# LouisNUST/pose-unsupervised

Hardware: AMD Instinct MI355X
Metric: 4-view 256x256 frames/sec (fwd+triangulate) (higher is better)
Workload: dtype bf16

## Files before the change

### include/posu.h

```cpp
#ifndef POSU_H_
#define POSU_H_

#ifdef __cplusplus
extern "C" {
#endif

#define POSU_OK 0
#define POSU_ERR_ARG 1
#define POSU_ERR_HIP 2

#define POSU_F32 0
#define POSU_BF16 1
#define POSU_F64 2
#define POSU_F16 3
#define POSU_F16X3 4

const char* posu_last_error(void);
int posu_abi_version(void);

int posu_pack_nchw_to_nhwc(int dtype, const float* x, int N, int C, int H, int W,
                           void* y, int Cpad, int hflip, void* stream);

int posu_pack_s2d_nchw(int dtype, const float* x, int N, int C, int H, int W,
                       void* y, int Cpad, int hflip, void* stream);
// ... 51 lines not shown
                                          const float* s2, const float* b2, const float* s3, const float* b3,
                                          void* y, const float* s1n, const float* b1n, void* t1n, void* stream);
int posu_bottleneck_down_tail_stream_fwd(int dtype, const void* t1, const void* x, int N, int H, int W, int C,
                                         int P, const void* wstream, long long wstream_bytes, const float* s2,
                                         const float* b2, const float* s3, const float* b3, void* y,
                                         const float* s1n, const float* b1n, void* t1n, void* stream);

int posu_bottleneck_s2_tail_fwd(int dtype, const void* t1, const void* x, int N, int H, int W, int C, int P,
                                const void* wstream, long long wstream_bytes, const float* s2, const float* b2,
                                const float* shift, int Cout, void* y, void* stream);

int posu_bottleneck_s2_tail_next_fwd(int dtype, const void* t1, const void* x, int N, int H, int W, int C, int P,
                                     const void* wstream, long long wstream_bytes, const float* s2, const float* b2,
                                     const float* shift, int Cout, void* y, const float* s1n, const float* b1n,
                                     void* t1n, void* stream);

int posu_bottleneck_down_fwd(int dtype, const void* x, int N, int H, int W, int C, int P,
                             const void* w1, const float* s1, const float* b1, const void* w2,
                             const float* s2, const float* b2, const void* w3d, const float* shift3,
                             void* y, void* stream);

int posu_pack_view_rows(int dtype, const float* src, int V, int M, int HW, void* dst, void* stream);
int posu_gemm_rows_f32(int dtype, const void* x, int M, int K, const void* wt, int Ncol, int vblk,
                       float* out, void* stream);

int posu_deconv4x4s2_head_fwd(int dtype, const void* x, int N, int H, int W, int C,
                              const void* w, int Cout, const float* scale, const float* shift,
                              void* y, const void* hw, const void* hw_lo, int J, const float* hbias,
                              float* hm, void* stream);

// ... 238 lines not shown
```

### pose-unsupervised_amd/csrc/tail_common.h

```cpp
#pragma once
#include <string>

#include "gemm_common.h"

namespace posu {
namespace {

struct TailGeom {
  const void* t1;
  const void* x;
  void* y;
  const uint4* wst;
  const float* s2;
  const float* b2;
  const float* s3;
  const float* b3;
  int N, H;
  const float* s1n;
  const float* b1n;
  void* t1n;
  long long wseg;
  int warm;
};

template <int D, int STEPS>
struct WStream {
  static constexpr int kD = D;
  const char* grp;
  int wlane;
  uint4 wa[D][2];
  __device__ __forceinline__ WStream(const uint4* wst, int cq, int lane)
      : grp(reinterpret_cast<const char*>(wst) + cq * (STEPS * 2 * 1024)), wlane(lane * 16) {}
  __device__ __forceinline__ const uint4* frag(int p, int j) const {
    return reinterpret_cast<const uint4*>(grp + (min(p, STEPS - 1) * 2 + j) * 1024 + wlane);
  }
  __device__ __forceinline__ void refill(int slot, int p) {
    wa[slot][0] = *frag(p, 0);
// ... 136 lines not shown
    } else {
#pragma unroll
      for (int i = 0; i < MT; ++i) {
#pragma unroll
        for (int j = 0; j < 2; ++j) O::mma(acc[i][j], ws.wa[s][j], b[d % NB][i]);
        if (NB == 1 && d + 1 < KT) b[0][i] = *at(i, d + 1);
      }
      ws.refill(s, p0 + d + kD);
    }
    __builtin_amdgcn_sched_barrier(0);
  }
}

inline int tail_operands(TailGeom& g, const std::string& what, const void* t1, const void* x, int N, int H,
                         const void* wstream, long long wstream_bytes, const float* s2, const float* b2,
                         const float* s3, const float* b3, void* y, const float* s1n, const float* b1n, void* t1n) {
  POSU_REQUIRE(t1 && x && wstream && s2 && b2 && b3 && y, what + ": null pointer");
  POSU_REQUIRE(x != y && t1 != y, what + ": the output must not alias an input");
  POSU_REQUIRE(!t1n || (s1n && b1n && t1n != y && t1n != x && t1n != t1),
               what + ": the next conv1 needs its BN and an output that aliases no other operand");
  g = TailGeom{t1, x, y, static_cast<const uint4*>(wstream), s2, b2, s3, b3, N, H, s1n, b1n, t1n, wstream_bytes / 64,
               warm_wgs(wstream_bytes)};
  return POSU_OK;
}

inline int tail_sizes(const TailGeom& g, const std::string& what, int hmult, long long act_bytes,
                      long long wstream_bytes, long long need) {
  POSU_REQUIRE(wstream_bytes == need, what + ": wstream holds " + std::to_string(wstream_bytes) + " bytes, the " +
                                          (g.t1n ? "chained" : "plain") + " tail reads " + std::to_string(need));
  POSU_REQUIRE(g.N > 0 && g.H > 0 && g.H % hmult == 0,
               what + ": H must be a positive multiple of " + std::to_string(hmult) + " (the tile rows)");
  POSU_REQUIRE(act_bytes < (1LL << 31) - 256, what + ": activation exceeds the 2 GiB addressing range");
  for (const void* p : {g.t1, g.x, static_cast<const void*>(g.y), static_cast<const void*>(g.wst),
                        static_cast<const void*>(g.s3), static_cast<const void*>(g.b3),
                        static_cast<const void*>(g.t1n), static_cast<const void*>(g.s1n),
                        static_cast<const void*>(g.b1n)})
    POSU_REQUIRE((reinterpret_cast<size_t>(p) & 15) == 0, what + ": pointers must be 16-byte aligned");
  return POSU_OK;
}

}
}
```

### pose-unsupervised_amd/csrc/tail_s2.hip

```cpp
#include "tail_common.h"

namespace posu {
namespace {

template <bool NEXT>
struct S2Cfg {
  static constexpr int kWin = 64, kC = 256, kP = 128, kCout = 512, kWout = 32;
  static constexpr int kRows = 4, kTW = 16, kNW = 4, kPx = kRows * kTW;
  static constexpr int kWR = 2 * kRows + 1, kWC = 2 * kTW + 1;
  static constexpr int kRowB = kP * 2;
  static constexpr int kXRowB = kC * 2;
  static constexpr int kWinInst = (kWR * kWC * kRowB + 1023) / 1024;
  static constexpr int kBN2 = kWinInst * 1024;
  static constexpr int kLds = kBN2 + 2 * kP * 4;
  static constexpr int kT2 = 0;
  static constexpr int kX = kT2 + kPx * kRowB;
  static constexpr int kShift = kX + kPx * kXRowB;
  static constexpr int kKT = kP / 32;
  static constexpr int kKX = kC / 32;
  static constexpr int kNC = kCout / (32 * kNW);
  static constexpr int kSteps2 = 9 * kKT, kStepsC = kKT + kKX + (NEXT ? kKT : 0);
  static constexpr int kSteps = kSteps2 + kNC * kStepsC;
  static constexpr int kYC = kShift + kCout * 4;
  static constexpr int kD = 4;
  static_assert(kYC + (NEXT ? kPx * kRowB : 0) <= kBN2, "t2, the x pixels, the shift (and the y chunk) fit over the window");
  static_assert(2 * kLds <= 160 * 1024, "two workgroups per CU");
  static_assert(kKT % kD == 0 && kKX % kD == 0 && kSteps2 % kD == 0 && kStepsC % kD == 0,
                "every block starts on ring slot 0");
};

template <typename T, bool NEXT>
__global__ __launch_bounds__(S2Cfg<NEXT>::kNW * 64, 2) void tail_s2_kernel(TailGeom g) {
  using O = Op<T>;
  using K = S2Cfg<NEXT>;
  constexpr int ES = 2, MT = K::kRows;
  __shared__ __attribute__((aligned(16))) char smem[K::kLds];
  const int tid = threadIdx.x;
  const int lane = tid & 63;
  const int r16 = lane & 15, q = lane >> 4;
  const int cq = __builtin_amdgcn_readfirstlane(tid >> 6);
  const unsigned lds0 = static_cast<unsigned>(reinterpret_cast<size_t>((__attribute__((address_space(3))) char*)smem));
  const int Hin = g.H, Hout = Hin / 2;
  const int tiles_x = K::kWout / K::kTW, tiles_y = Hout / K::kRows;
  const int n = blockIdx.x / (tiles_x * tiles_y);
  const int rem = blockIdx.x - n * tiles_x * tiles_y;
  const int R0 = (rem / tiles_x) * K::kRows, C0 = (rem % tiles_x) * K::kTW;
  float* bn2 = reinterpret_cast<float*>(smem + K::kBN2);
  for (int c = tid; c < K::kP; c += K::kNW * 64) {
    bn2[c] = g.s2[c];
    bn2[K::kP + c] = g.b2[c];
  }

  {
    const u32x4 t1s = make_srd(g.t1, g.N * Hin * K::kWin * K::kP * ES);
    const int sub = lane >> 4, pc = lane & 15;
#pragma unroll
    for (int k = 0; k < (K::kWinInst + K::kNW - 1) / K::kNW; ++k) {
      const int m = cq + K::kNW * k;
      if (m < K::kWinInst) {
        const int pix = 4 * m + sub;
        const int wr = pix / K::kWC, wc = pix - wr * K::kWC;
        const int yy = 2 * R0 - 1 + wr, xx = 2 * C0 - 1 + wc;
        const int lc = pc ^ (wc & 15);
        const bool ok = wr < K::kWR && static_cast<unsigned>(yy) < static_cast<unsigned>(Hin) &&
                        static_cast<unsigned>(xx) < static_cast<unsigned>(K::kWin);
        dma16(t1s, ok ? (((n * Hin + yy) * K::kWin + xx) * K::kP + 8 * lc) * ES : kOOB,
              lds0 + static_cast<unsigned>(m) * 1024u);
      }
    }
  }

  WStream<K::kD, K::kSteps> ws(g.wst, cq, lane);
  ws.start(g, K::kNW * 64);

  f32x4 acc[MT][2];
  f32x4 acc1[MT][2];
  const int c32 = 32 * cq + cpair(q);
  using Win = Stride2Addr<K::kRowB, K::kWC>;
  using T2 = RowsAddr<K::kRowB, K::kTW, K::kTW>;
  using XI = RowsAddr<K::kXRowB, K::kTW, K::kTW>;

  zero(acc);
#pragma unroll 1
  for (int t = 0; t < 9; ++t) {
    const int dy = t / 3, dx = t - 3 * (t / 3);
    kblock<O, K::kKT, 2>(acc, ws, K::kKT * t, Win(smem, dy, dx, r16, q));
  }
  lds_barrier();
  {
    const u32x4 xs = make_srd(g.x, g.N * Hin * K::kWin * K::kC * ES);
    const int sub = lane >> 5, pc = lane & 31;
#pragma unroll
    for (int k = 0; k < K::kPx / 2 / K::kNW; ++k) {
      const int m = cq + K::kNW * k;
      const int px = 2 * m + sub, i = px >> 4, r = px & 15;
      const int lc = (pc & 16) | ((pc ^ r) & 15);
      dma16(xs, (((n * Hin + 2 * (R0 + i)) * K::kWin + 2 * (C0 + r)) * K::kC + 8 * lc) * ES,
            lds0 + static_cast<unsigned>(K::kX + m * 1024));
    }
  }
  {
// ... 6 lines not shown
    for (int i = 0; i < MT; ++i) {
      float v[8];
      pair(acc, i, v);
      bn_relu(v, sc, sh, nullptr);
      lds_store8<O, K::kRowB>(smem + K::kT2, 16 * i + r16, r16, c32 >> 3, v);
    }
  }
  vm_wait<0>();
  lds_barrier();

  const float* shl = reinterpret_cast<const float*>(smem + K::kShift);
  T* yg = reinterpret_cast<T*>(g.y);
  if constexpr (NEXT) zero(acc1);
#pragma unroll
  for (int nc = 0; nc < K::kNC; ++nc) {
    const int p0 = K::kSteps2 + K::kStepsC * nc;
    zero(acc);
    kblock<O, K::kKT, 2>(acc, ws, p0, T2(smem + K::kT2, r16, r16, q));
    kblock<O, K::kKX, 2>(acc, ws, p0 + K::kKT, XI(smem + K::kX, r16, r16, q));
    const int c0 = 128 * nc + c32;
    float sh[8];
    ld8(shl + c0, sh);
    if constexpr (NEXT) {
      if (nc > 0) lds_barrier();
    }
#pragma unroll
    for (int i = 0; i < MT; ++i) {
      float v[8];
      pair(acc, i, v);
      add8<false>(v, sh);
#pragma unroll
// ... 17 lines not shown
      float v[8];
      pair(acc1, i, v);
      bn_relu(v, sc, sh, nullptr);
      const size_t pix = (static_cast<size_t>(n) * Hout + R0 + i) * K::kWout + C0 + r16;
      *reinterpret_cast<uint4*>(tg + pix * K::kP + c32) = O::store_vals(v);
    }
  }
}

}
}

using namespace posu;

namespace {
int s2_tail_impl(const char* name, int dtype, const void* t1, const void* x, int N, int H, int W, int C, int P,
                 const void* wstream, long long wstream_bytes, const float* s2, const float* b2, const float* shift,
                 int Cout, void* y, const float* s1n, const float* b1n, void* t1n, void* stream) {
  const std::string what = name;
  const bool next = t1n != nullptr;
  using K = S2Cfg<false>;
  POSU_REQUIRE(dtype == POSU_BF16 || dtype == POSU_F16, what + ": dtype must be BF16 or F16");
  TailGeom g;
  if (int e = tail_operands(g, what, t1, x, N, H, wstream, wstream_bytes, s2, b2, nullptr, shift, y, s1n, b1n, t1n))
    return e;
  POSU_REQUIRE(W == K::kWin && C == K::kC && P == K::kP && Cout == K::kCout,
               what + ": built for the first Bottleneck of layer2 of PoseResNet at 256x256 (input W = 64, C = 256, "
                      "planes = 128, output channels 512)");
  const long long need = static_cast<long long>(K::kNW) * (next ? S2Cfg<true>::kSteps : K::kSteps) * 2 * 1024;
  if (int e = tail_sizes(g, what, 2 * K::kRows, static_cast<long long>(N) * H * W * C * 2, wstream_bytes, need))
    return e;
  const dim3 grid(static_cast<unsigned>(N * (H / 2 / K::kRows) * (K::kWout / K::kTW)));
  hipStream_t s = as_stream(stream);
  if (dtype == POSU_BF16) {
    if (next) hipLaunchKernelGGL((tail_s2_kernel<uint16_t, true>), grid, dim3(K::kNW * 64), 0, s, g);
    else hipLaunchKernelGGL((tail_s2_kernel<uint16_t, false>), grid, dim3(K::kNW * 64), 0, s, g);
  } else {
    if (next) hipLaunchKernelGGL((tail_s2_kernel<f16_t, true>), grid, dim3(K::kNW * 64), 0, s, g);
    else hipLaunchKernelGGL((tail_s2_kernel<f16_t, false>), grid, dim3(K::kNW * 64), 0, s, g);
  }
  return check_launch(name);
}
}

extern "C" int posu_bottleneck_s2_tail_fwd(int dtype, const void* t1, const void* x, int N, int H, int W, int C,
                                           int P, const void* wstream, long long wstream_bytes, const float* s2,
                                           const float* b2, const float* shift, int Cout, void* y, void* stream) {
  return s2_tail_impl("posu_bottleneck_s2_tail_fwd", dtype, t1, x, N, H, W, C, P, wstream, wstream_bytes, s2, b2,
                      shift, Cout, y, nullptr, nullptr, nullptr, stream);
}

extern "C" int posu_bottleneck_s2_tail_next_fwd(int dtype, const void* t1, const void* x, int N, int H, int W, int C,
                                                int P, const void* wstream, long long wstream_bytes, const float* s2,
                                                const float* b2, const float* shift, int Cout, void* y,
                                                const float* s1n, const float* b1n, void* t1n, void* stream) {
  if (!t1n) {
    set_error("posu_bottleneck_s2_tail_next_fwd: null pointer (t1n)");
    return POSU_ERR_ARG;
  }
  return s2_tail_impl("posu_bottleneck_s2_tail_next_fwd", dtype, t1, x, N, H, W, C, P, wstream, wstream_bytes, s2,
                      b2, shift, Cout, y, s1n, b1n, t1n, stream);
}
```

### pose-unsupervised_amd/lib/posu/_native.py

```python
import ctypes
import os
import threading

import torch

F32 = 0
BF16 = 1
F64 = 2
F16 = 3
F16X3 = 4

ABI_VERSION = 16

_LIB_PATH = os.path.join(os.path.dirname(os.path.abspath(__file__)), 'libposeu.so')
_lock = threading.Lock()
_lib = None

_p = ctypes.c_void_p
_i = ctypes.c_int
_f = ctypes.c_float
_ll = ctypes.c_longlong
_d = ctypes.c_double

_SIGNATURES = {
# ... 6 lines not shown
    'posu_nhwc_to_nchw_f32': [_i, _p, _i, _i, _i, _i, _p, _p],
    'posu_conv1x1_dual_fwd': [_i, _p, _i, _i, _i, _i, _p, _i, _i, _i, _i, _p, _i, _p, _p, _i, _p, _i, _p],
    'posu_conv_bk': [_i],
    'posu_stem_pool_fwd': [_i, _p, _i, _i, _i, _i, _p, _p, _p, _p, _p],
    'posu_stem_pool_views_fwd': [_i, _p, _i, _i, _i, _i, _i, _p, _p, _p, _p, _p],
    'posu_bottleneck_fwd': [_i, _p, _i, _i, _i, _i, _i, _p, _p, _p, _p, _p, _p, _p, _p, _p, _p, _p],
    'posu_bottleneck_tail_stream_fwd': [_i, _p, _p, _i, _i, _i, _i, _i, _p, _ll, _p, _p, _p, _p, _p, _p],
    'posu_bottleneck_tail_stream_next_fwd': [_i, _p, _p, _i, _i, _i, _i, _i, _p, _ll, _p, _p, _p, _p, _p, _p, _p,
                                             _p, _p],
    'posu_bottleneck_tail_stream_chain_fwd': [_i, _p, _p, _i, _i, _i, _i, _i, _i, _p, _ll, _p, _p, _p, _p, _p, _p,
                                              _p, _p, _p],
    'posu_bottleneck_down_tail_stream_fwd': [_i, _p, _p, _i, _i, _i, _i, _i, _p, _ll, _p, _p, _p, _p, _p, _p, _p,
                                             _p, _p],
    'posu_bottleneck_s2_tail_fwd': [_i, _p, _p, _i, _i, _i, _i, _i, _p, _ll, _p, _p, _p, _i, _p, _p],
    'posu_bottleneck_s2_tail_next_fwd': [_i, _p, _p, _i, _i, _i, _i, _i, _p, _ll, _p, _p, _p, _i, _p, _p, _p, _p, _p],
    'posu_bottleneck_down_fwd': [_i, _p, _i, _i, _i, _i, _i, _p, _p, _p, _p, _p, _p, _p, _p, _p, _p],
    'posu_conv2d_fwd': [_i, _p, _i, _i, _i, _i, _p, _i, _i, _i, _i, _i, _p, _p, _p, _i, _p, _i, _i, _i, _p],
    'posu_deconv4x4s2_fwd': [_i, _p, _i, _i, _i, _i, _p, _i, _p, _p, _i, _p, _i, _p],
    'posu_deconv4x4s2_head_fwd': [_i, _p, _i, _i, _i, _i, _p, _i, _p, _p, _p, _p, _p, _i, _p, _p, _p],
    'posu_head1x1_nchw_fwd': [_i, _p, _i, _i, _i, _i, _p, _i, _p, _p, _p],
    'posu_maxpool3x3s2_fwd': [_i, _p, _i, _i, _i, _i, _p, _p],
    'posu_softargmax2d_fwd': [_p, _i, _i, _i, _i, _f, _p, _p, _p, _p],
    'posu_softargmax2d_bwd': [_p, _p, _i, _i, _i, _i, _f, _p, _p, _p, _p],
    'posu_argmax2d_fwd': [_p, _i, _i, _i, _i, _i, _p, _p, _p, _p],
    'posu_affine2d_apply': [_p, _p, _i, _i, _i, _p, _p],
    'posu_epipolar_loss_fwd': [_p, _p, _p, _p, _i, _i, _i, _i, _p, _p, _p],
    'posu_epipolar_loss_bwd': [_p, _p, _p, _p, _i, _i, _i, _i, _p, _p, _p],
    'posu_triangulate_dlt': [_p, _p, _p, _i, _i, _i, _p, _i, _i, _i, _i, _p, _p],
    'posu_joints_mse_fwd': [_p, _p, _p, _i, _i, _i, _p, _p, _p],
    'posu_joints_mse_bwd': [_p, _p, _p, _i, _i, _i, _p, _p, _p],
# ... 138 lines not shown
```

### pose-unsupervised_amd/lib/posu/ops.py

```python
import numpy as np
import torch

from . import _native as nat
from ._native import F32, BF16, F64, F16, F16X3, ptr, call, stream_of, require_cuda

_TORCH_OF = {F32: torch.float32, BF16: torch.bfloat16, F16: torch.float16, F16X3: torch.float16}


def dtype_code(dtype):
    if dtype in ('bf16', torch.bfloat16, BF16):
        return BF16
    if dtype in ('fp32', 'f32', torch.float32, F32):
        return F32
    if dtype in ('fp16', 'f16', torch.float16, F16):
        return F16
    if dtype in ('fp16x3', F16X3):
        return F16X3
    raise ValueError('unsupported compute dtype %r (bf16 | fp16 | fp16x3 | fp32)' % (dtype,))


def torch_dtype(code):
    return _TORCH_OF[code]


# ... 99 lines not shown
    call('posu_bottleneck_s2_tail_fwd', code, ptr(t1), ptr(x), n, h, w, c, t1.shape[3], ptr(wstream),
         wstream.numel() * wstream.element_size(), ptr(s2), ptr(b2), ptr(shift), shift.numel(), ptr(out),
         stream_of(x.device))
    return out


def bottleneck_s2_tail_next_nhwc(t1, x, wstream, s2, b2, shift, s1n, b1n, code, out=None, t1n=None):
    n, h, w, c = x.shape
    if out is None:
        out = torch.empty((n, h // 2, w // 2, shift.numel()), dtype=x.dtype, device=x.device)
    if t1n is None:
        t1n = torch.empty((n, h // 2, w // 2, s1n.numel()), dtype=x.dtype, device=x.device)
    call('posu_bottleneck_s2_tail_next_fwd', code, ptr(t1), ptr(x), n, h, w, c, t1.shape[3], ptr(wstream),
         wstream.numel() * wstream.element_size(), ptr(s2), ptr(b2), ptr(shift), shift.numel(), ptr(out), ptr(s1n),
         ptr(b1n), ptr(t1n), stream_of(x.device))
    return out, t1n


def bottleneck_tail_stream_next_nhwc(t1, x, wstream, s2, b2, s3, b3, s1n, b1n, code, out=None, t1n=None):
    n, h, w, c = x.shape
    p = t1.shape[3]
    if out is None:
        out = torch.empty_like(x)
    if t1n is None:
        t1n = torch.empty((n, h, w, p), dtype=x.dtype, device=x.device)
    cm = cmul(code)
    call('posu_bottleneck_tail_stream_next_fwd', code, ptr(t1), ptr(x), n, h, w, c // cm, p // cm, ptr(wstream),
         wstream.numel() * wstream.element_size(), ptr(s2), ptr(b2), ptr(s3), ptr(b3), ptr(out), ptr(s1n), ptr(b1n),
         ptr(t1n), stream_of(x.device))
    return out, t1n
# ... 855 lines not shown
```

### pose-unsupervised_amd/lib/posu/packing.py

```python
import numpy as np
import torch

COUT_ALIGN = 64


def round_up(x, m):
    return (x + m - 1) // m * m


def pack_conv_weight(w, cin_pad, bk, dtype):
    cout, cin, kh, kw = w.shape
    k = kh * kw * cin_pad
    wt = torch.zeros((cout, kh, kw, cin_pad), dtype=torch.float32, device=w.device)
    wt[..., :cin] = w.detach().float().permute(0, 2, 3, 1)
    out = torch.zeros((round_up(cout, COUT_ALIGN), round_up(k, bk)), dtype=torch.float32, device=w.device)
    out[:cout, :k] = wt.reshape(cout, k)
    return out.to(dtype).contiguous()


def mfma_fragments(wpk):
    co, k = wpk.shape
    return wpk.reshape(co // 16, 16, k // 32, 4, 8).permute(0, 2, 3, 1, 4).reshape(co // 16, k // 32, 64, 8)


def pack_s2_tail_stream(w2pk, wdual, w1n=None):
    if tuple(w2pk.shape) != (128, 1152) or tuple(wdual.shape) != (512, 384):
        raise ValueError('pack_s2_tail_stream: conv2 pack [128][1152] and dual pack [512][384] expected, got %s / %s'
                         % (tuple(w2pk.shape), tuple(wdual.shape)))
    f2 = mfma_fragments(w2pk)
    s2 = f2.reshape(4, 2, 36, 64, 8).permute(0, 2, 1, 3, 4)
    fd = mfma_fragments(wdual)
    sd = fd.reshape(4, 4, 2, 12, 64, 8).permute(1, 0, 3, 2, 4, 5)
    if w1n is None:
        return torch.cat([s2, sd.reshape(4, 48, 2, 64, 8)], dim=1).contiguous()
    if tuple(w1n.shape) != (128, 512):
        raise ValueError('pack_s2_tail_stream: the next conv1 pack must be [128][512], got %s' % (tuple(w1n.shape),))
    f1 = mfma_fragments(w1n)
    s1 = f1.reshape(4, 2, 4, 4, 64, 8).permute(0, 2, 3, 1, 4, 5)
    sdn = torch.cat([sd, s1], dim=2)
    return torch.cat([s2, sdn.reshape(4, 64, 2, 64, 8)], dim=1).contiguous()


def pack_tail_stream(w2pk, w3pk, w1n=None):
# ... 232 lines not shown
```

### pose-unsupervised_amd/lib/posu/plan.py

```python
from collections import namedtuple

import torch

from . import ops
from .packing import (fold_bn, pack_bottleneck_conv1_weight, pack_bottleneck_conv3_weight, pack_bottleneck_down_weight,
                      pack_conv_weight, pack_deconv4x4_weight, pack_down_tail_stream,
                      pack_dual_1x1_weight, pack_s2_tail_stream, pack_stem_fused_weight, pack_stem_s2d_weight,
                      pack_tail_stream, split_exponent, to_split)

STEM_CIN_PAD = 8
STEM_S2D_PAD = 16
SPLIT_PAD = 32


def _stem_pads(code):
    return (2 * SPLIT_PAD, SPLIT_PAD) if code == ops.F16X3 else (STEM_CIN_PAD, STEM_S2D_PAD)


def _pack(pk32, code):
    if code == ops.F16X3:
        e = split_exponent(pk32)
        return to_split(pk32, e), e
    return pk32.to(ops.torch_dtype(code)).contiguous(), 0

# ... 145 lines not shown
        self.scale = None if e == 0 else torch.full((self.cout,), 2.0 ** -e, device=self.shift.device)
        self.stride2 = dconv.stride[0]

    def __call__(self, mid, x, code, out=None):
        if out is None:
            out = torch.empty(tuple(mid.shape[:3]) + (self.cout * ops.cmul(code),), dtype=mid.dtype, device=mid.device)
        key = ('dual', code, tuple(mid.shape), tuple(x.shape), self.cout)
        return _tuned(key, self.cout, lambda t: ops.conv1x1_dual_nhwc(
            mid, x, self.stride2, self.w, self.cout, self.shift, True, code, out=out, tile=t, scale=self.scale))


FUSED_BOTTLENECK = True
S2_TAIL = True
CHAINED_TAILS = True
S2_CHAIN = True
TAIL_W24 = True
SPLIT_TAILS = True
TAIL_W96 = True
CHAIN_LAYERS = True
CHAIN_LAYERS_2B = False
CHUNKS_F16X3 = 2
EARLY_LAYERS = 2
_FUSED_MAX_BYTES = (1 << 31) - 256


def _fused_fits(x, cout):
    px = x.shape[0] * x.shape[1] * x.shape[2]
    es = x.element_size()
    return px * max(x.shape[3], cout) * es < _FUSED_MAX_BYTES

# ... 41 lines not shown
        ds = blk.downsample
        if ds is not None and len(names) == 3 and ds[0].kernel_size == (1, 1) and \
                blk.conv3.weight.shape[1] % bk == 0 and ds[0].weight.shape[1] % bk == 0:
            for nm in names[:2]:
                self.convs.append(_Conv(getattr(blk, nm), getattr(blk, 'bn' + nm[-1]), True, code, bk))
            self.dual = _DualTail(blk.conv3, blk.bn3, ds[0], ds[1], code)
            c2 = self.convs[1]
            if self._built_for('fused_down'):
                self.packs['fused_down'] = pack_bottleneck_down_weight(self.dual.w, 64)
            if self._built_for('down_tail'):
                self.packs['down_tail'] = pack_down_tail_stream(c2.w, self.dual.w)
                self.dscale = (self.dual.scale if self.dual.scale is not None else
                               torch.ones(self.dual.cout, device=self.dual.shift.device))
            if self._built_for('s2_tail'):
                self.packs['s2_tail'] = pack_s2_tail_stream(c2.w, self.dual.w)
            return
        for nm in names:
            self.convs.append(_Conv(getattr(blk, nm), getattr(blk, 'bn' + nm[-1]), True, code, bk))
        if ds is not None:
            self.down = _Conv(ds[0], ds[1], False, code, bk)
        if self._built_for('fused'):
            self.packs['fused'] = (pack_bottleneck_conv1_weight(blk.conv1.weight, ops.torch_dtype(code)),
                                   pack_bottleneck_conv3_weight(blk.conv3.weight, ops.torch_dtype(code)))
        self.kind = next((k for k in ('l1', 'l2', 'l3') if self._built_for(k)), None)
        if self.kind is not None:
            self.packs['tail'] = pack_tail_stream(self.convs[1].w, self.convs[2].w)

    def _built_for(self, kernel):
        g = _GEOMETRY[kernel]
        if self.down is not None or (self.dual is None) != (g.dual is None) or len(self.convs) != (2 if g.dual else 3):
# ... 10 lines not shown
    def _chains(self, how):
        return self.kind is not None and any(self.code in a.codes and how in a.chains
                                             for a in _GEOMETRY[self.kind].at)

    def link_next(self, nxt):
        c2 = self.convs[1]
        if self.kind is not None and self.kind == nxt.kind:
            self.chain = nxt.convs[0]
            self.packs['tail_next'] = pack_tail_stream(c2.w, self.convs[2].w, self.chain.w)
        elif 'down_tail' in self.packs and nxt.kind == 'l1':
            self.chain = nxt.convs[0]
            self.packs['down_tail_next'] = pack_down_tail_stream(c2.w, self.dual.w, self.chain.w)
        elif 's2_tail' in self.packs and nxt.kind == 'l2':
            self.chain = nxt.convs[0]
            self.packs['s2_tail_next'] = pack_s2_tail_stream(c2.w, self.dual.w, self.chain.w)

    def link_layer(self, first):
        if not (self._chains('layer') and (self.code in _SPLIT or CHAIN_LAYERS_2B) and first.dual is not None):
            return
        c1n = first.convs[0]
        planes = self.convs[1].cout
        if c1n.k == 1 and c1n.stride == 1 and c1n.cout == 2 * planes and tuple(c1n.w.shape)[1] == self.convs[0].w.shape[1]:
            self.xchain = c1n
            self.packs['tail_layer'] = pack_tail_stream(self.convs[1].w, self.convs[2].w, c1n.w)

    @property
    def cout(self):
        return self.dual.cout if self.dual is not None else self.convs[-1].cout

    def _at(self, kernel, x):
# ... 47 lines not shown
            c1, c2, c3 = cs
            w1f, w3f = self.packs['fused']
            return ops.bottleneck_nhwc(x, w1f, c1.scale, c1.shift, c2.w, c2.scale, c2.shift, w3f, c3.scale, c3.shift,
                                       code, out=out), None
        if variant == 'fused_down':
            c1, c2 = cs
            return ops.bottleneck_down_nhwc(x, c1.w, c1.scale, c1.shift, c2.w, c2.scale, c2.shift,
                                            self.packs['fused_down'], self.dual.shift, code, out=out), None
        if variant == 'down_tail':
            c1, c2 = cs
            s1n, b1n = (self.chain.scale, self.chain.shift) if chained else (None, None)
            return ops.bottleneck_down_tail_stream_nhwc(
                c1(x, code), x, self.packs['down_tail_next' if chained else 'down_tail'], c2.scale, c2.shift,
                self.dscale, self.dual.shift, code, s1n=s1n, b1n=b1n, out=out)
        if variant == 's2_tail':
            c1, c2 = cs
            if chained:
                n1 = self.chain
                return ops.bottleneck_s2_tail_next_nhwc(c1(x, code), x, self.packs['s2_tail_next'], c2.scale, c2.shift,
                                                        self.dual.shift, n1.scale, n1.shift, code, out=out)
            return ops.bottleneck_s2_tail_nhwc(c1(x, code), x, self.packs['s2_tail'], c2.scale, c2.shift,
                                               self.dual.shift, code, out=out), None
        if variant == 'dual':
            return self.dual(cs[1](cs[0](x, code) if t1 is None else t1, code), x, code, out=out), None
        res = self.down(x, code) if self.down is not None else x
        y = x
        for c in cs[:-1]:
            y = c(y, code)
        return cs[-1](y, code, residual=res, out=out), None

    def __call__(self, x, code, out=None):
        return self.run(x, code, out=out, chain=False)[0]


class _Deconv:
    __slots__ = ('w', 'scale', 'shift', 'cout')

    def __init__(self, dc, bn, code, bk):
        if dc.stride != (2, 2) or dc.padding != (1, 1) or dc.output_padding != (0, 0):
            raise NotImplementedError('deconv supported for kernel 4, stride 2, padding 1')
        self.w, e = _pack(pack_deconv4x4_weight(dc.weight, 32 if code == ops.F16X3 else bk, torch.float32), code)
        self.scale, self.shift = fold_bn(bn, dc.bias)
        self.scale = _unscale(self.scale, e)
        self.cout = dc.weight.shape[1]
# ... 235 lines not shown
```

### pose-unsupervised_amd/lib/posu/roofline.py

```python

_R50 = ((3, 64, 64, 256, 64), (4, 128, 256, 512, 64), (6, 256, 512, 1024, 32), (3, 512, 1024, 2048, 16))


def r50_256_launches(n=128, es=2, joints=17):
    out = []
    act = lambda hw, c: n * hw * hw * c * es
    wb = lambda *dims: es * _prod(dims)
    out.append(('stem_pool (4 views)', n * 3 * 256 * 256 * 4 + wb(64, 147), act(64, 64)))
    out.append(('layer1.0 bottleneck64 (down)', act(64, 64) + wb(64, 64) + wb(64, 576) + wb(256, 64) + wb(256, 64),
                act(64, 256)))
    for b in (1, 2):
        out.append(('layer1.%d bottleneck64' % b, act(64, 256) + wb(64, 256) + wb(64, 576) + wb(256, 64),
                    act(64, 256)))
    out.append(('layer2.0 conv1', act(64, 256) + wb(128, 256), act(64, 128)))
    out.append(('layer2.0 strided tail + layer2.1 conv1',
                act(64, 128) + act(32, 256) + wb(128, 1152) + wb(512, 384) + wb(128, 512),
                act(32, 512) + act(32, 128)))
    for b in (1, 2):
        out.append(('layer2.%d chained tail' % b, act(32, 128) + act(32, 512) + wb(128, 1152) + wb(512, 128) +
                    wb(128, 512), act(32, 512) + act(32, 128)))
    out.append(('layer2.3 tail', act(32, 128) + act(32, 512) + wb(128, 1152) + wb(512, 128), act(32, 512)))
    out.append(('layer3.0 conv1', act(32, 512) + wb(256, 512), act(32, 256)))
    out.append(('layer3.0 conv2 s2', act(32, 256) + wb(256, 2304), act(16, 256)))
    out.append(('layer3.0 conv3|down', act(16, 256) + act(16, 512) + wb(1024, 768), act(16, 1024)))
    out.append(('layer3.1 conv1', act(16, 1024) + wb(256, 1024), act(16, 256)))
    for b in (1, 2, 3, 4):
        out.append(('layer3.%d chained tail' % b, act(16, 256) + act(16, 1024) + wb(256, 2304) + wb(1024, 256) +
                    wb(256, 1024), act(16, 1024) + act(16, 256)))
    out.append(('layer3.5 tail', act(16, 256) + act(16, 1024) + wb(256, 2304) + wb(1024, 256), act(16, 1024)))
    out.append(('layer4.0 conv1', act(16, 1024) + wb(512, 1024), act(16, 512)))
    out.append(('layer4.0 conv2 s2', act(16, 512) + wb(512, 4608), act(8, 512)))
    out.append(('layer4.0 conv3|down', act(8, 512) + act(8, 1024) + wb(2048, 1536), act(8, 2048)))
# ... 90 lines not shown
```

Measured before the change: 56530.

## Fuse layer2.0 conv1 into the strided tail kernel with autotuned selection

Result: faster. 58010 (median of 6 runs) (+2.6%).

```diff
diff --git a/include/posu.h b/include/posu.h
--- a/include/posu.h
+++ b/include/posu.h
@@ -89,6 +89,16 @@
                                      const void* wstream, long long wstream_bytes, const float* s2, const float* b2,
                                      const float* shift, int Cout, void* y, const float* s1n, const float* b1n,
                                      void* t1n, void* stream);
+
+int posu_bottleneck_s2_front_tail_fwd(int dtype, const void* x, int N, int H, int W, int C, int P, const float* s1,
+                                      const float* b1, const void* wstream, long long wstream_bytes,
+                                      const float* s2, const float* b2, const float* shift, int Cout, void* y,
+                                      void* stream);
+int posu_bottleneck_s2_front_tail_next_fwd(int dtype, const void* x, int N, int H, int W, int C, int P,
+                                           const float* s1, const float* b1, const void* wstream,
+                                           long long wstream_bytes, const float* s2, const float* b2,
+                                           const float* shift, int Cout, void* y, const float* s1n,
+                                           const float* b1n, void* t1n, void* stream);
 
 int posu_bottleneck_down_fwd(int dtype, const void* x, int N, int H, int W, int C, int P,
                              const void* w1, const float* s1, const float* b1, const void* w2,
diff --git a/pose-unsupervised_amd/csrc/tail_common.h b/pose-unsupervised_amd/csrc/tail_common.h
--- a/pose-unsupervised_amd/csrc/tail_common.h
+++ b/pose-unsupervised_amd/csrc/tail_common.h
@@ -21,6 +21,8 @@
   void* t1n;
   long long wseg;
   int warm;
+  const float* s1;
+  const float* b1;
 };
 
 template <int D, int STEPS>
@@ -187,13 +189,14 @@
 
 inline int tail_operands(TailGeom& g, const std::string& what, const void* t1, const void* x, int N, int H,
                          const void* wstream, long long wstream_bytes, const float* s2, const float* b2,
-                         const float* s3, const float* b3, void* y, const float* s1n, const float* b1n, void* t1n) {
-  POSU_REQUIRE(t1 && x && wstream && s2 && b2 && b3 && y, what + ": null pointer");
+                         const float* s3, const float* b3, void* y, const float* s1n, const float* b1n, void* t1n,
+                         bool front = false, const float* s1 = nullptr, const float* b1 = nullptr) {
+  POSU_REQUIRE((front ? s1 && b1 : t1 != nullptr) && x && wstream && s2 && b2 && b3 && y, what + ": null pointer");
   POSU_REQUIRE(x != y && t1 != y, what + ": the output must not alias an input");
   POSU_REQUIRE(!t1n || (s1n && b1n && t1n != y && t1n != x && t1n != t1),
                what + ": the next conv1 needs its BN and an output that aliases no other operand");
   g = TailGeom{t1, x, y, static_cast<const uint4*>(wstream), s2, b2, s3, b3, N, H, s1n, b1n, t1n, wstream_bytes / 64,
-               warm_wgs(wstream_bytes)};
+               warm_wgs(wstream_bytes), s1, b1};
   return POSU_OK;
 }
 
@@ -207,7 +210,8 @@
   for (const void* p : {g.t1, g.x, static_cast<const void*>(g.y), static_cast<const void*>(g.wst),
                         static_cast<const void*>(g.s3), static_cast<const void*>(g.b3),
                         static_cast<const void*>(g.t1n), static_cast<const void*>(g.s1n),
-                        static_cast<const void*>(g.b1n)})
+                        static_cast<const void*>(g.b1n), static_cast<const void*>(g.s1),
+                        static_cast<const void*>(g.b1)})
     POSU_REQUIRE((reinterpret_cast<size_t>(p) & 15) == 0, what + ": pointers must be 16-byte aligned");
   return POSU_OK;
 }
diff --git a/pose-unsupervised_amd/csrc/tail_s2.hip b/pose-unsupervised_amd/csrc/tail_s2.hip
--- a/pose-unsupervised_amd/csrc/tail_s2.hip
+++ b/pose-unsupervised_amd/csrc/tail_s2.hip
@@ -3,7 +3,7 @@
 namespace posu {
 namespace {
 
-template <bool NEXT>
+template <bool NEXT, bool FRONT = false>
 struct S2Cfg {
   static constexpr int kWin = 64, kC = 256, kP = 128, kCout = 512, kWout = 32;
   static constexpr int kRows = 4, kTW = 16, kNW = 4, kPx = kRows * kTW;
@@ -20,19 +20,32 @@
   static constexpr int kKX = kC / 32;
   static constexpr int kNC = kCout / (32 * kNW);
   static constexpr int kSteps2 = 9 * kKT, kStepsC = kKT + kKX + (NEXT ? kKT : 0);
-  static constexpr int kSteps = kSteps2 + kNC * kStepsC;
+  static constexpr int kF = FRONT ? kKX : 0;
+  static constexpr int kWinPx = kWinInst * 1024 / kRowB, kGroups = (kWR * kWC + 16 * kRows - 1) / (16 * kRows);
+  static constexpr int kSteps = kF + kSteps2 + kNC * kStepsC;
   static constexpr int kYC = kShift + kCout * 4;
   static constexpr int kD = 4;
   static_assert(kYC + (NEXT ? kPx * kRowB : 0) <= kBN2, "t2, the x pixels, the shift (and the y chunk) fit over the window");
   static_assert(2 * kLds <= 160 * 1024, "two workgroups per CU");
-  static_assert(kKT % kD == 0 && kKX % kD == 0 && kSteps2 % kD == 0 && kStepsC % kD == 0,
+  static_assert(kKT % kD == 0 && kKX % kD == 0 && kSteps2 % kD == 0 && kStepsC % kD == 0 && kF % kD == 0,
                 "every block starts on ring slot 0");
 };
 
-template <typename T, bool NEXT>
+template <int KX>
+struct HeldW {
+  static constexpr int kD = KX;
+  uint4 wa[KX][2];
+  __device__ __forceinline__ void refill(int, int) {}
+};
+template <int RowB>
+__device__ __forceinline__ uint4* win_chunk(char* img, int pix, int wc, int c8) {
+  return reinterpret_cast<uint4*>(img + pix * RowB + ((c8 ^ (wc & 15)) << 4));
+}
+
+template <typename T, bool NEXT, bool FRONT = false>
 __global__ __launch_bounds__(S2Cfg<NEXT>::kNW * 64, 2) void tail_s2_kernel(TailGeom g) {
   using O = Op<T>;
-  using K = S2Cfg<NEXT>;
+  using K = S2Cfg<NEXT, FRONT>;
   constexpr int ES = 2, MT = K::kRows;
   __shared__ __attribute__((aligned(16))) char smem[K::kLds];
   const int tid = threadIdx.x;
@@ -51,7 +64,7 @@
     bn2[K::kP + c] = g.b2[c];
   }
 
-  {
+  if constexpr (!FRONT) {
     const u32x4 t1s = make_srd(g.t1, g.N * Hin * K::kWin * K::kP * ES);
     const int sub = lane >> 4, pc = lane & 15;
 #pragma unroll
@@ -71,20 +84,106 @@
   }
 
   WStream<K::kD, K::kSteps> ws(g.wst, cq, lane);
-  ws.start(g, K::kNW * 64);
+  if constexpr (!FRONT) ws.start(g, K::kNW * 64);
 
   f32x4 acc[MT][2];
   f32x4 acc1[MT][2];
   const int c32 = 32 * cq + cpair(q);
+
   using Win = Stride2Addr<K::kRowB, K::kWC>;
   using T2 = RowsAddr<K::kRowB, K::kTW, K::kTW>;
   using XI = RowsAddr<K::kXRowB, K::kTW, K::kTW>;
+
+  if constexpr (FRONT) {
+    constexpr int kGrpPx = 16 * MT, kGrpB = kGrpPx * K::kXRowB;
+    constexpr int kDma = kGrpB / 1024 / K::kNW;
+    static_assert(2 * kGrpB <= (K::kGroups - 1) * kGrpPx * K::kRowB, "both buffers below the last group's t1");
+    static_assert(K::kGroups * kGrpPx >= K::kWinPx, "the groups cover the window");
+    unsigned wv[kWarmLoads];
+    warm_issue(wv, g.wst, g.wseg, g.warm, K::kNW * 64);
+    HeldW<K::kKX> w1;
+#pragma unroll
+    for (int d = 0; d < K::kKX; ++d)
+#pragma unroll
+      for (int j = 0; j < 2; ++j) w1.wa[d][j] = *ws.frag(d, j);
+    float sc[8], sh[8];
+    ld8(g.s1 + c32, sc);
+    ld8(g.b1 + c32, sh);
+    const u32x4 xs = make_srd(g.x, g.N * Hin * K::kWin * K::kC * ES);
+    auto px_off = [&](int pix, int& wc) {
+      const int wr = pix / K::kWC;
+      wc = pix - wr * K::kWC;
+      const int yy = 2 * R0 - 1 + wr, xx = 2 * C0 - 1 + wc;
+      const bool ok = wr < K::kWR && static_cast<unsigned>(yy) < static_cast<unsigned>(Hin) &&
+                      static_cast<unsigned>(xx) < static_cast<unsigned>(K::kWin);
+      return ok ? ((n * Hin + yy) * K::kWin + xx) * K::kC * ES : kOOB;
+    };
+    auto stage = [&](int gr, int b) {
+      const int sub = lane >> 5, pc = lane & 31;
+#pragma unroll
+      for (int k = 0; k < kDma; ++k) {
+        const int m = cq + K::kNW * k;
+        const int px = 2 * m + sub, r = px & 15;
+        const int lc = (pc & 16) | ((pc ^ r) & 15);
+        int wc;
+        const int off = px_off(kGrpPx * gr + px, wc);
+        dma16(xs, off == kOOB ? kOOB : off + 8 * lc * ES, lds0 + static_cast<unsigned>(b * kGrpB + m * 1024));
+      }
+    };
+    warm_use(wv);
+#pragma unroll
+    for (int d = 0; d < K::kKX; ++d) asm volatile("" ::"v"(w1.wa[d][0].x), "v"(w1.wa[d][1].x));
+    asm volatile("" ::"v"(sc[0]), "v"(sc[4]), "v"(sh[0]), "v"(sh[4]));
+    stage(K::kGroups - 1, 0);
+    stage(K::kGroups - 2, 1);
+    uint4 held[K::kGroups][MT];
+#pragma unroll
+    for (int s = 0; s < K::kGroups; ++s) {
+      const int gr = K::kGroups - 1 - s;
+      if (s + 1 < K::kGroups) vm_wait<kDma>();
+      else vm_wait<0>();
+      lds_barrier();
+      zero(acc);
+      kblock<O, K::kKX, 2>(acc, w1, 0, XI(smem + (s & 1) * kGrpB, r16, r16, q));
+      lds_barrier();
+      if (s + 2 < K::kGroups) stage(gr - 2, s & 1);
+#pragma unroll
+      for (int i = 0; i < MT; ++i) {
+        float v[8];
+        pair(acc, i, v);
+        bn_relu(v, sc, sh, nullptr);
+        int wc;
+        const bool pad = px_off(kGrpPx * gr + 16 * i + r16, wc) == kOOB;
+#pragma unroll
+        for (int e = 0; e < 8; ++e) v[e] = pad ? 0.f : v[e];
+        held[s][i] = O::store_vals(v);
+      }
+      if (s == 0) {
+#pragma unroll
+        for (int i = 0; i < MT; ++i) {
+          const int pix = kGrpPx * gr + 16 * i + r16;
+          if (pix < K::kWinPx) *win_chunk<K::kRowB>(smem, pix, pix % K::kWC, c32 >> 3) = held[s][i];
+        }
+      }
+    }
+#pragma unroll
+    for (int d = 0; d < K::kD; ++d) ws.refill(d, K::kF + d);
+#pragma unroll
+    for (int s = 1; s < K::kGroups; ++s)
+#pragma unroll
+      for (int i = 0; i < MT; ++i) {
+        const int pix = kGrpPx * (K::kGroups - 1 - s) + 16 * i + r16;
+        *win_chunk<K::kRowB>(smem, pix, pix % K::kWC, c32 >> 3) = held[s][i];
+      }
+    vm_wait<0>();
+    lds_barrier();
+  }
 
   zero(acc);
 #pragma unroll 1
   for (int t = 0; t < 9; ++t) {
     const int dy = t / 3, dx = t - 3 * (t / 3);
-    kblock<O, K::kKT, 2>(acc, ws, K::kKT * t, Win(smem, dy, dx, r16, q));
+    kblock<O, K::kKT, 2>(acc, ws, K::kF + K::kKT * t, Win(smem, dy, dx, r16, q));
   }
   lds_barrier();
   {
@@ -121,7 +220,7 @@
   if constexpr (NEXT) zero(acc1);
 #pragma unroll
   for (int nc = 0; nc < K::kNC; ++nc) {
-    const int p0 = K::kSteps2 + K::kStepsC * nc;
+    const int p0 = K::kF + K::kSteps2 + K::kStepsC * nc;
     zero(acc);
     kblock<O, K::kKT, 2>(acc, ws, p0, T2(smem + K::kT2, r16, r16, q));
     kblock<O, K::kKX, 2>(acc, ws, p0 + K::kKT, XI(smem + K::kX, r16, r16, q));
@@ -169,31 +268,40 @@
 using namespace posu;
 
 namespace {
-int s2_tail_impl(const char* name, int dtype, const void* t1, const void* x, int N, int H, int W, int C, int P,
-                 const void* wstream, long long wstream_bytes, const float* s2, const float* b2, const float* shift,
-                 int Cout, void* y, const float* s1n, const float* b1n, void* t1n, void* stream) {
+template <typename T>
+void s2_launch(bool next, bool front, dim3 grid, dim3 block, hipStream_t s, const TailGeom& g) {
+  if (front) {
+    if (next) hipLaunchKernelGGL((tail_s2_kernel<T, true, true>), grid, block, 0, s, g);
+    else hipLaunchKernelGGL((tail_s2_kernel<T, false, true>), grid, block, 0, s, g);
+  } else {
+    if (next) hipLaunchKernelGGL((tail_s2_kernel<T, true>), grid, block, 0, s, g);
+    else hipLaunchKernelGGL((tail_s2_kernel<T, false>), grid, block, 0, s, g);
+  }
+}
+
+int s2_tail_impl(const char* name, int dtype, bool front, const void* t1, const float* s1, const float* b1,
+                 const void* x, int N, int H, int W, int C, int P, const void* wstream, long long wstream_bytes,
+                 const float* s2, const float* b2, const float* shift, int Cout, void* y, const float* s1n,
+                 const float* b1n, void* t1n, void* stream) {
   const std::string what = name;
   const bool next = t1n != nullptr;
   using K = S2Cfg<false>;
   POSU_REQUIRE(dtype == POSU_BF16 || dtype == POSU_F16, what + ": dtype must be BF16 or F16");
   TailGeom g;
-  if (int e = tail_operands(g, what, t1, x, N, H, wstream, wstream_bytes, s2, b2, nullptr, shift, y, s1n, b1n, t1n))
+  if (int e = tail_operands(g, what, t1, x, N, H, wstream, wstream_bytes, s2, b2, nullptr, shift, y, s1n, b1n, t1n,
+                            front, s1, b1))
     return e;
   POSU_REQUIRE(W == K::kWin && C == K::kC && P == K::kP && Cout == K::kCout,
                what + ": built for the first Bottleneck of layer2 of PoseResNet at 256x256 (input W = 64, C = 256, "
                       "planes = 128, output channels 512)");
-  const long long need = static_cast<long long>(K::kNW) * (next ? S2Cfg<true>::kSteps : K::kSteps) * 2 * 1024;
+  const int steps = (next ? S2Cfg<true>::kSteps : K::kSteps) + (front ? S2Cfg<false, true>::kF : 0);
+  const long long need = static_cast<long long>(K::kNW) * steps * 2 * 1024;
   if (int e = tail_sizes(g, what, 2 * K::kRows, static_cast<long long>(N) * H * W * C * 2, wstream_bytes, need))
     return e;
   const dim3 grid(static_cast<unsigned>(N * (H / 2 / K::kRows) * (K::kWout / K::kTW)));
   hipStream_t s = as_stream(stream);
-  if (dtype == POSU_BF16) {
-    if (next) hipLaunchKernelGGL((tail_s2_kernel<uint16_t, true>), grid, dim3(K::kNW * 64), 0, s, g);
-    else hipLaunchKernelGGL((tail_s2_kernel<uint16_t, false>), grid, dim3(K::kNW * 64), 0, s, g);
-  } else {
-    if (next) hipLaunchKernelGGL((tail_s2_kernel<f16_t, true>), grid, dim3(K::kNW * 64), 0, s, g);
-    else hipLaunchKernelGGL((tail_s2_kernel<f16_t, false>), grid, dim3(K::kNW * 64), 0, s, g);
-  }
+  if (dtype == POSU_BF16) s2_launch<uint16_t>(next, front, grid, dim3(K::kNW * 64), s, g);
+  else s2_launch<f16_t>(next, front, grid, dim3(K::kNW * 64), s, g);
   return check_launch(name);
 }
 }
@@ -201,8 +309,8 @@
 extern "C" int posu_bottleneck_s2_tail_fwd(int dtype, const void* t1, const void* x, int N, int H, int W, int C,
                                            int P, const void* wstream, long long wstream_bytes, const float* s2,
                                            const float* b2, const float* shift, int Cout, void* y, void* stream) {
-  return s2_tail_impl("posu_bottleneck_s2_tail_fwd", dtype, t1, x, N, H, W, C, P, wstream, wstream_bytes, s2, b2,
-                      shift, Cout, y, nullptr, nullptr, nullptr, stream);
+  return s2_tail_impl("posu_bottleneck_s2_tail_fwd", dtype, false, t1, nullptr, nullptr, x, N, H, W, C, P, wstream,
+                      wstream_bytes, s2, b2, shift, Cout, y, nullptr, nullptr, nullptr, stream);
 }
 
 extern "C" int posu_bottleneck_s2_tail_next_fwd(int dtype, const void* t1, const void* x, int N, int H, int W, int C,
@@ -213,6 +321,27 @@
     set_error("posu_bottleneck_s2_tail_next_fwd: null pointer (t1n)");
     return POSU_ERR_ARG;
   }
-  return s2_tail_impl("posu_bottleneck_s2_tail_next_fwd", dtype, t1, x, N, H, W, C, P, wstream, wstream_bytes, s2,
-                      b2, shift, Cout, y, s1n, b1n, t1n, stream);
-}
+  return s2_tail_impl("posu_bottleneck_s2_tail_next_fwd", dtype, false, t1, nullptr, nullptr, x, N, H, W, C, P,
+                      wstream, wstream_bytes, s2, b2, shift, Cout, y, s1n, b1n, t1n, stream);
+}
+
+extern "C" int posu_bottleneck_s2_front_tail_fwd(int dtype, const void* x, int N, int H, int W, int C, int P,
+                                                 const float* s1, const float* b1, const void* wstream,
+                                                 long long wstream_bytes, const float* s2, const float* b2,
+                                                 const float* shift, int Cout, void* y, void* stream) {
+  return s2_tail_impl("posu_bottleneck_s2_front_tail_fwd", dtype, true, nullptr, s1, b1, x, N, H, W, C, P, wstream,
+                      wstream_bytes, s2, b2, shift, Cout, y, nullptr, nullptr, nullptr, stream);
+}
+
+extern "C" int posu_bottleneck_s2_front_tail_next_fwd(int dtype, const void* x, int N, int H, int W, int C, int P,
+                                                      const float* s1, const float* b1, const void* wstream,
+                                                      long long wstream_bytes, const float* s2, const float* b2,
+                                                      const float* shift, int Cout, void* y, const float* s1n,
+                                                      const float* b1n, void* t1n, void* stream) {
+  if (!t1n) {
+    set_error("posu_bottleneck_s2_front_tail_next_fwd: null pointer (t1n)");
+    return POSU_ERR_ARG;
+  }
+  return s2_tail_impl("posu_bottleneck_s2_front_tail_next_fwd", dtype, true, nullptr, s1, b1, x, N, H, W, C, P,
+                      wstream, wstream_bytes, s2, b2, shift, Cout, y, s1n, b1n, t1n, stream);
+}
diff --git a/pose-unsupervised_amd/lib/posu/_native.py b/pose-unsupervised_amd/lib/posu/_native.py
--- a/pose-unsupervised_amd/lib/posu/_native.py
+++ b/pose-unsupervised_amd/lib/posu/_native.py
@@ -44,6 +44,9 @@
                                              _p, _p],
     'posu_bottleneck_s2_tail_fwd': [_i, _p, _p, _i, _i, _i, _i, _i, _p, _ll, _p, _p, _p, _i, _p, _p],
     'posu_bottleneck_s2_tail_next_fwd': [_i, _p, _p, _i, _i, _i, _i, _i, _p, _ll, _p, _p, _p, _i, _p, _p, _p, _p, _p],
+    'posu_bottleneck_s2_front_tail_fwd': [_i, _p, _i, _i, _i, _i, _i, _p, _p, _p, _ll, _p, _p, _p, _i, _p, _p],
+    'posu_bottleneck_s2_front_tail_next_fwd': [_i, _p, _i, _i, _i, _i, _i, _p, _p, _p, _ll, _p, _p, _p, _i, _p, _p, _p,
+                                               _p, _p],
     'posu_bottleneck_down_fwd': [_i, _p, _i, _i, _i, _i, _i, _p, _p, _p, _p, _p, _p, _p, _p, _p, _p],
     'posu_conv2d_fwd': [_i, _p, _i, _i, _i, _i, _p, _i, _i, _i, _i, _i, _p, _p, _p, _i, _p, _i, _i, _i, _p],
     'posu_deconv4x4s2_fwd': [_i, _p, _i, _i, _i, _i, _p, _i, _p, _p, _i, _p, _i, _p],
diff --git a/pose-unsupervised_amd/lib/posu/ops.py b/pose-unsupervised_amd/lib/posu/ops.py
--- a/pose-unsupervised_amd/lib/posu/ops.py
+++ b/pose-unsupervised_amd/lib/posu/ops.py
@@ -137,6 +137,28 @@
     call('posu_bottleneck_s2_tail_next_fwd', code, ptr(t1), ptr(x), n, h, w, c, t1.shape[3], ptr(wstream),
          wstream.numel() * wstream.element_size(), ptr(s2), ptr(b2), ptr(shift), shift.numel(), ptr(out), ptr(s1n),
          ptr(b1n), ptr(t1n), stream_of(x.device))
+    return out, t1n
+
+
+def bottleneck_s2_front_tail_nhwc(x, s1, b1, wstream, s2, b2, shift, code, out=None):
+    n, h, w, c = x.shape
+    if out is None:
+        out = torch.empty((n, h // 2, w // 2, shift.numel()), dtype=x.dtype, device=x.device)
+    call('posu_bottleneck_s2_front_tail_fwd', code, ptr(x), n, h, w, c, s2.numel(), ptr(s1), ptr(b1), ptr(wstream),
+         wstream.numel() * wstream.element_size(), ptr(s2), ptr(b2), ptr(shift), shift.numel(), ptr(out),
+         stream_of(x.device))
+    return out
+
+
+def bottleneck_s2_front_tail_next_nhwc(x, s1, b1, wstream, s2, b2, shift, s1n, b1n, code, out=None, t1n=None):
+    n, h, w, c = x.shape
+    if out is None:
+        out = torch.empty((n, h // 2, w // 2, shift.numel()), dtype=x.dtype, device=x.device)
+    if t1n is None:
+        t1n = torch.empty((n, h // 2, w // 2, s1n.numel()), dtype=x.dtype, device=x.device)
+    call('posu_bottleneck_s2_front_tail_next_fwd', code, ptr(x), n, h, w, c, s2.numel(), ptr(s1), ptr(b1),
+         ptr(wstream), wstream.numel() * wstream.element_size(), ptr(s2), ptr(b2), ptr(shift), shift.numel(),
+         ptr(out), ptr(s1n), ptr(b1n), ptr(t1n), stream_of(x.device))
     return out, t1n
 
 
diff --git a/pose-unsupervised_amd/lib/posu/packing.py b/pose-unsupervised_amd/lib/posu/packing.py
--- a/pose-unsupervised_amd/lib/posu/packing.py
+++ b/pose-unsupervised_amd/lib/posu/packing.py
@@ -23,10 +23,17 @@
     return wpk.reshape(co // 16, 16, k // 32, 4, 8).permute(0, 2, 3, 1, 4).reshape(co // 16, k // 32, 64, 8)
 
 
-def pack_s2_tail_stream(w2pk, wdual, w1n=None):
+def pack_s2_tail_stream(w2pk, wdual, w1n=None, w1=None):
     if tuple(w2pk.shape) != (128, 1152) or tuple(wdual.shape) != (512, 384):
         raise ValueError('pack_s2_tail_stream: conv2 pack [128][1152] and dual pack [512][384] expected, got %s / %s'
                          % (tuple(w2pk.shape), tuple(wdual.shape)))
+    if w1 is not None:
+        if tuple(w1.shape) != (128, 256):
+            raise ValueError('pack_s2_tail_stream: the block\'s conv1 pack must be [128][256], got %s' % (tuple(w1.shape),))
+        if w1.dtype != w2pk.dtype:
+            raise ValueError('pack_s2_tail_stream: the conv1 pack is %s, the conv2 pack %s' % (w1.dtype, w2pk.dtype))
+        ff = mfma_fragments(w1).reshape(4, 2, 8, 64, 8).permute(0, 2, 1, 3, 4)
+        return torch.cat([ff, pack_s2_tail_stream(w2pk, wdual, w1n)], dim=1).contiguous()
     f2 = mfma_fragments(w2pk)
     s2 = f2.reshape(4, 2, 36, 64, 8).permute(0, 2, 1, 3, 4)
     fd = mfma_fragments(wdual)
diff --git a/pose-unsupervised_amd/lib/posu/plan.py b/pose-unsupervised_amd/lib/posu/plan.py
--- a/pose-unsupervised_amd/lib/posu/plan.py
+++ b/pose-unsupervised_amd/lib/posu/plan.py
@@ -183,6 +183,8 @@
 S2_TAIL = True
 CHAINED_TAILS = True
 S2_CHAIN = True
+S2_FRONT = False
+S2_FRONT_TUNE = True
 TAIL_W24 = True
 SPLIT_TAILS = True
 TAIL_W96 = True
@@ -254,6 +256,7 @@
                                torch.ones(self.dual.cout, device=self.dual.shift.device))
             if self._built_for('s2_tail'):
                 self.packs['s2_tail'] = pack_s2_tail_stream(c2.w, self.dual.w)
+                self.packs['s2_front'] = pack_s2_tail_stream(c2.w, self.dual.w, w1=self.convs[0].w)
             return
         for nm in names:
             self.convs.append(_Conv(getattr(blk, nm), getattr(blk, 'bn' + nm[-1]), True, code, bk))
@@ -294,6 +297,7 @@
         elif 's2_tail' in self.packs and nxt.kind == 'l2':
             self.chain = nxt.convs[0]
             self.packs['s2_tail_next'] = pack_s2_tail_stream(c2.w, self.dual.w, self.chain.w)
+            self.packs['s2_front_next'] = pack_s2_tail_stream(c2.w, self.dual.w, self.chain.w, w1=self.convs[0].w)
 
     def link_layer(self, first):
         if not (self._chains('layer') and (self.code in _SPLIT or CHAIN_LAYERS_2B) and first.dual is not None):
@@ -371,13 +375,8 @@
                 c1(x, code), x, self.packs['down_tail_next' if chained else 'down_tail'], c2.scale, c2.shift,
                 self.dscale, self.dual.shift, code, s1n=s1n, b1n=b1n, out=out)
         if variant == 's2_tail':
-            c1, c2 = cs
-            if chained:
-                n1 = self.chain
-                return ops.bottleneck_s2_tail_next_nhwc(c1(x, code), x, self.packs['s2_tail_next'], c2.scale, c2.shift,
-                                                        self.dual.shift, n1.scale, n1.shift, code, out=out)
-            return ops.bottleneck_s2_tail_nhwc(c1(x, code), x, self.packs['s2_tail'], c2.scale, c2.shift,
-                                               self.dual.shift, code, out=out), None
+            front = S2_FRONT or (S2_FRONT_TUNE and self._front_tuned(x, code, chained, out))
+            return self._s2_tail(x, code, chained, out, front)
         if variant == 'dual':
             return self.dual(cs[1](cs[0](x, code) if t1 is None else t1, code), x, code, out=out), None
         res = self.down(x, code) if self.down is not None else x
@@ -385,6 +384,44 @@
         for c in cs[:-1]:
             y = c(y, code)
         return cs[-1](y, code, residual=res, out=out), None
+
+    def _s2_tail(self, x, code, chained, out, front):
+        c1, c2 = self.convs
+        n1 = self.chain
+        if front:
+            if chained:
+                return ops.bottleneck_s2_front_tail_next_nhwc(
+                    x, c1.scale, c1.shift, self.packs['s2_front_next'], c2.scale, c2.shift, self.dual.shift,
+                    n1.scale, n1.shift, code, out=out)
+            return ops.bottleneck_s2_front_tail_nhwc(x, c1.scale, c1.shift, self.packs['s2_front'], c2.scale,
+                                                     c2.shift, self.dual.shift, code, out=out), None
+        if chained:
+            return ops.bottleneck_s2_tail_next_nhwc(c1(x, code), x, self.packs['s2_tail_next'], c2.scale, c2.shift,
+                                                    self.dual.shift, n1.scale, n1.shift, code, out=out)
+        return ops.bottleneck_s2_tail_nhwc(c1(x, code), x, self.packs['s2_tail'], c2.scale, c2.shift,
+                                           self.dual.shift, code, out=out), None
+
+    def _front_tuned(self, x, code, chained, out):
+        key = ('s2_front', code, tuple(x.shape), bool(chained))
+        if _Tuner.active and key not in _TUNE_CACHE:
+            seen = list(_Tuner.seen)
+            times = {}
+            for order in ((0, 1), (1, 0)):
+                for f in order:
+                    self._s2_tail(x, code, chained, out, bool(f))
+                    a, b = torch.cuda.Event(enable_timing=True), torch.cuda.Event(enable_timing=True)
+                    a.record()
+                    for _ in range(_Tuner.reps):
+                        self._s2_tail(x, code, chained, out, bool(f))
+                    b.record()
+                    b.synchronize()
+                    ms = a.elapsed_time(b)
+                    times[f] = min(ms, times.get(f, ms))
+            _TUNE_CACHE[key] = int(times[1] < times[0])
+            _TUNE_TIMES[key] = times
+            if _TUNE_CACHE[key]:
+                _Tuner.seen[:] = seen
+        return bool(_TUNE_CACHE.get(key, 0))
 
     def __call__(self, x, code, out=None):
         return self.run(x, code, out=out, chain=False)[0]
diff --git a/pose-unsupervised_amd/lib/posu/roofline.py b/pose-unsupervised_amd/lib/posu/roofline.py
--- a/pose-unsupervised_amd/lib/posu/roofline.py
+++ b/pose-unsupervised_amd/lib/posu/roofline.py
@@ -2,7 +2,7 @@
 _R50 = ((3, 64, 64, 256, 64), (4, 128, 256, 512, 64), (6, 256, 512, 1024, 32), (3, 512, 1024, 2048, 16))
 
 
-def r50_256_launches(n=128, es=2, joints=17):
+def r50_256_launches(n=128, es=2, joints=17, s2_front=False):
     out = []
     act = lambda hw, c: n * hw * hw * c * es
     wb = lambda *dims: es * _prod(dims)
@@ -12,10 +12,15 @@
     for b in (1, 2):
         out.append(('layer1.%d bottleneck64' % b, act(64, 256) + wb(64, 256) + wb(64, 576) + wb(256, 64),
                     act(64, 256)))
-    out.append(('layer2.0 conv1', act(64, 256) + wb(128, 256), act(64, 128)))
-    out.append(('layer2.0 strided tail + layer2.1 conv1',
-                act(64, 128) + act(32, 256) + wb(128, 1152) + wb(512, 384) + wb(128, 512),
-                act(32, 512) + act(32, 128)))
+    if s2_front:
+        out.append(('layer2.0 conv1 + strided tail + layer2.1 conv1',
+                    act(64, 256) + wb(128, 256) + wb(128, 1152) + wb(512, 384) + wb(128, 512),
+                    act(32, 512) + act(32, 128)))
+    else:
+        out.append(('layer2.0 conv1', act(64, 256) + wb(128, 256), act(64, 128)))
+        out.append(('layer2.0 strided tail + layer2.1 conv1',
+                    act(64, 128) + act(32, 256) + wb(128, 1152) + wb(512, 384) + wb(128, 512),
+                    act(32, 512) + act(32, 128)))
     for b in (1, 2):
         out.append(('layer2.%d chained tail' % b, act(32, 128) + act(32, 512) + wb(128, 1152) + wb(512, 128) +
                     wb(128, 512), act(32, 512) + act(32, 128)))
```
